# alvin-zyl/LDDL

Measured on AMD Instinct MI355X. Metric: WordPiece tokens/sec (node) BERT seq128/512 at 1-8 GPUs; % HBM roofline, higher is better.
Workload: dtype u8

## Files before the change

lddl_amd/csrc/capi.hip:

```cpp
#include "capi_ctx.h"

static thread_local char g_err[1024];

int set_err(int code, const char* fmt, ...) {
  va_list ap;
  va_start(ap, fmt);
  vsnprintf(g_err, sizeof g_err, fmt, ap);
  va_end(ap);
  return code;
}

extern "C" const char* lddl_last_error(void) { return g_err; }

static void free_ctx(lddl_ctx* c) {
  if (!c) return;
  (void)hipFree(c->d_tdbg);
  (void)hipFree(c->d_pdbg);
  (void)hipFree(c->d_top);
  (void)hipFree(c->d_pages);
  (void)hipFree(c->d_bmp);
  (void)hipFree(c->d_xmap);
  (void)hipFree(c->d_multi);
  (void)hipFree(c->d_slots);
  (void)hipFree(c->d_bloom);
// ... 149 lines not shown
}

extern "C" int lddl_tokenize_stats(lddl_ctx* c, double* out, int n) {
  if (!c || !out || n < 6) return set_err(LDDL_EINVAL, "need out[6]");
  if (!c->timing || !c->tm) return set_err(LDDL_EINVAL, "timing is off (lddl_set_timing)");
  HIP_TRY(hipSetDevice(c->device));
  for (int k = 0; k < 3; ++k) {
    double ms = 0.0;
    for (int i = 0; i < c->tm->n[k]; ++i) {
      HIP_TRY(hipEventSynchronize(c->tm->ev[k][1][i]));
      float f = 0.0f;
      HIP_TRY(hipEventElapsedTime(&f, c->tm->ev[k][0][i], c->tm->ev[k][1][i]));
      ms += f;
    }
    out[k] = ms;
  }
  unsigned long long nrec = 0;
  HIP_TRY(hipMemcpy(&nrec, c->d_nrec, 8, hipMemcpyDeviceToHost));
  out[3] = (double)nrec;
  out[4] = (double)c->tm->n[0];
  uint32_t nfb = 0;
  HIP_TRY(hipMemcpy(&nfb, c->d_counter + 8, 4, hipMemcpyDeviceToHost));
  out[5] = (double)nfb;
  return 0;
}
```

lddl_amd/csrc/capi_ctx.h:

```cpp
#pragma once
#include <hip/hip_runtime.h>

#include <stdarg.h>
#include <stdint.h>
#include <stdio.h>
#include <stdlib.h>
#include <string.h>

#include <algorithm>
#include <new>
#include <string>
#include <vector>

#include "../../include/lddl_amd.h"
#include "collate.h"
#include "common.h"
#include "pack.h"
#include "render.h"
#include "tok_tables.h"
#include "tokenize.h"

using namespace lddl;

__attribute__((visibility("hidden"))) int set_err(int code, const char* fmt, ...);
// ... 45 lines not shown

enum CtxWs {
  CW_BIN_HIST,
  CW_BIN_BASE,
  CW_BIN_BSUM,
  CW_BIN_ERR,
  CW_NPY_ERR,
  CW_TILE_SENT,
  CW_FB_LIST,
  CW_FB_COUNT,
  CW_ENT,
  CW_SHARED_ROWS,
  CW_SHARED_BSUM,
  CW_SHARED_META,
  CW_COLLATE_ERR,
  CW_SENT_SPEC,
  CW_PCS,
  CW_SNSLOT,
  CW_CNT8,
  CW_SCAN_BSUM,
  CW_PCH,
  CW_CHUNK_PART,
  CW_PART_PB,
  CW_COUNT
};

enum HostWord {
  HW_NPAIRS,
  HW_BART_LO = HW_NPAIRS,
  HW_NTOK,
  HW_BART_HI = HW_NTOK,
  HW_PACK_ERR,
  HW_BART_NSENT = HW_PACK_ERR,
  HW_NMASK,
  HW_MARENA_USED,
  HW_NDENSE,
  HW_CU_TOTAL = HW_NDENSE,
  HW_MAX_LEN,
  HW_RENDER_BYTES = HW_MAX_LEN,
  HW_ERR,
  HW_COUNT
};
static_assert(HW_MAX_LEN == HW_CU_TOTAL + 1, "lddl_collate_rows_cu_seqlens reads total and max_len with one copy");
static_assert(HW_PACK_ERR == HW_NTOK + 1 && HW_NMASK == HW_NTOK + 2, "lddl_rows_from_strings_len reads its three totals with one copy");

struct lddl_pack {
  int device = 0;
  WsBuf ws[PW_COUNT];
  PackParams pp{};
  int64_t last_npairs = -1, last_ntok = -1, last_nmask = -1, last_ndense = 0;
  int pack_codebert = 0;
  uint64_t mlm_cap = 0;
  uint16_t* last_tokens = nullptr;
// ... 18 lines not shown
  uint8_t* d_pool = nullptr;
  uint32_t* d_voff = nullptr;
  uint8_t* d_rpool = nullptr;
  uint32_t* d_rinfo = nullptr;
  uint32_t maxb[2] = {0, 0};
  uint4* d_vt = nullptr;
  uint32_t vt_mask = 0;
  uint32_t* d_vbloom = nullptr;
  bool scan_ok = false;
  bool timing = false;
  SplitTiming* tm = nullptr;
  unsigned long long* d_nrec = nullptr;
  const void* spec_ids = nullptr;
  const void* spec_ntok = nullptr;
  const void* spec_soff = nullptr;
  int64_t spec_nsent = -1;
  bool spec_flags = false;
  WsBuf ws[CW_COUNT];
  int64_t* h_tot = nullptr;
  lddl_pack own;
  uint64_t mlm_cap0 = 0;
  int tok_grid = 0;
  int tok_algo = 5;
  uint8_t* d_ovf = nullptr;
  uint32_t* d_counter = nullptr;
  uint64_t* d_tdbg = nullptr;
  uint64_t* d_pdbg = nullptr;
  int64_t pdbg_cap = 0;
  uint2* d_ctab = nullptr;
  uint32_t ctab_mask = 0;
};

template <class T>
static int ws_get(WsBuf* ws, int slot, size_t n, T** out) {
  auto& b = ws[slot];
  const size_t bytes = (n ? n : 1) * sizeof(T);
  if (b.cap < bytes) {
    (void)hipFree(b.p);
    b.p = nullptr;
    b.cap = 0;
    HIP_TRY(hipMalloc(&b.p, bytes));
    b.cap = bytes;
  }
  *out = (T*)b.p;
  return 0;
}
// ... 29 lines not shown
```

lddl_amd/csrc/capi_tokenize.hip:

```cpp
#include "capi_ctx.h"

static int tok_debug_report(const TokParams& P, int64_t nt, hipStream_t st) {
  uint64_t h[24];
  HIP_TRY(hipMemcpyAsync(h, P.dbg, sizeof h, hipMemcpyDeviceToHost, st));
  HIP_TRY(hipStreamSynchronize(st));
  const char* nm[12] = {"loop", "setup", "classify", "except", "units", "urec", "prep", "probe", "records",
                        "tile_end", "entries", "tiles"};
  fprintf(stderr, "[lddl tok5 dbg] ntiles=%lld", (long long)nt);
  for (int k = 0; k < 12; ++k) fprintf(stderr, " %s=%llu", nm[k], (unsigned long long)h[k]);
  const char* wn[6] = {"wp_A", "wp_B", "wp_C", "wp_D", "wp_steps", "wp_lane_steps"};
  for (int k = 0; k < 6; ++k) fprintf(stderr, " %s=%llu", wn[k], (unsigned long long)h[12 + k]);
  fprintf(stderr, " prep_decode=%llu prep_dirty=%llu x_list=%llu x_load=%llu x_apply=%llu", (unsigned long long)h[18],
          (unsigned long long)h[19], (unsigned long long)h[20], (unsigned long long)h[21], (unsigned long long)h[22]);
  fprintf(stderr, "\n");
  return 0;
}

extern "C" int lddl_tokenize(lddl_ctx* c, const uint8_t* d_bytes, int64_t nbytes, const int64_t* d_sent_off,
                             int64_t n_sent, int32_t max_tok, uint16_t* d_out_ids, int64_t out_cap,
                             int32_t* d_out_ntok, int64_t* d_out_tok_off, void* stream) {
  if (!c) return set_err(LDDL_EINVAL, "null ctx");
  if (n_sent < 0 || max_tok < 1 || max_tok > 65534 || nbytes < 0 || out_cap < 0)
    return set_err(LDDL_EINVAL, "n_sent %lld nbytes %lld max_tok %d out_cap %lld", (long long)n_sent,
                   (long long)nbytes, max_tok, (long long)out_cap);
// ... 34 lines not shown
  P.bloom = c->d_bloom;
  P.pool = c->d_pool;
  P.voff = c->d_voff;
  P.maxb[0] = c->maxb[0];
  P.maxb[1] = c->maxb[1];
  for (int k = 0; k < 5; ++k) P.special[k] = c->special[k];
  P.unk = c->special[1];
  P.vt = c->d_vt;
  P.vt_mask = c->vt_mask;
  P.vbloom = c->d_vbloom;
  P.ovf = c->d_ovf;
  P.work_counter = c->d_counter;
  HIP_TRY(hipMemsetAsync(c->d_counter, 0, 64, st));
  const char* dbgenv = getenv("LDDL_TOK_DEBUG");

  if (dbgenv && dbgenv[0] == '1') {
    if (!c->d_tdbg) HIP_TRY(hipMalloc((void**)&c->d_tdbg, 32 * 8));
    HIP_TRY(hipMemsetAsync(c->d_tdbg, 0, 32 * 8, st));
    P.dbg = c->d_tdbg;
  }
  const int64_t nt = tile_count(nbytes);
  const char* eseg = getenv("LDDL_SPLIT_SEG");
  const char* ech = getenv("LDDL_SPLIT_CHUNKS");
  const int64_t seg_max = c->tok_algo == 0 ? nt : eseg && atoll(eseg) > 0 ? atoll(eseg) : SPLIT_SEG_TILES;
  const int64_t seg = nt < seg_max ? nt : seg_max;
  const bool split = c->tok_algo == 5;
  int64_t n_chunks = !split ? 1 : split_seg_slots(seg, c->n_cu) / SPLIT_CHUNK;
  if (ech && atoll(ech) > 0 && split) n_chunks = atoll(ech);
  const int64_t slots = n_chunks * SPLIT_CHUNK;
  int64_t* tile_sent;
  SplitParams S{};
  int rc;
  const int64_t fb_cap = fb_list_cap(seg, n_sent);
  if ((rc = ws_get(c, CW_TILE_SENT, nt + 1, &tile_sent)) || (rc = ws_get(c, CW_FB_LIST, (size_t)(2 * fb_cap), &S.fb_list)) ||
      (rc = ws_get(c, CW_FB_COUNT, 16, &S.fb_count)) ||
      (rc = ws_get(c, CW_ENT, (size_t)seg * 1024 + (size_t)max_tok + 4096, &S.ent)) ||
      (rc = ws_get(c, CW_SHARED_BSUM, (size_t)n_chunks + 16, &S.chunk_fill)) ||
      (rc = ws_get(c, CW_SCAN_BSUM, (size_t)scan_blocks(n_sent) + 1, &S.scan_bsum)))
    return rc;
  if ((rc = ws_get(c, CW_SHARED_ROWS, (size_t)slots * 4, &S.rec)) || (rc = ws_get(c, CW_PCS, (size_t)slots * 4, &S.pcs)) ||
      (rc = ws_get(c, CW_PCH, (size_t)slots, &S.pch)) || (rc = ws_get(c, CW_SHARED_META, n_sent, &S.smeta)) ||
      (rc = ws_get(c, CW_SNSLOT, n_sent, &S.snslot)) || (rc = ws_get(c, CW_CNT8, (size_t)slots, &S.cnt8)))
    return rc;
  if (!S.pch || !S.smeta || !S.snslot || !S.cnt8 || !S.rec || !S.pcs)
    return set_err(LDDL_EINVAL, "tokenize: finish scratch not allocated");
  S.chunk_ctr = S.chunk_fill + n_chunks;
  S.n_chunks = (uint32_t)n_chunks;
  S.seg_tiles = seg;
  S.fb_cap = fb_cap;
  S.seg_sent_cap = n_sent;
  S.n_fallback = c->d_counter + 8;
  if (c->timing) {
    S.n_rec = c->d_nrec;
    HIP_TRY(hipMemsetAsync(c->d_nrec, 0, 8, st));
  }
  if (c->tok_algo == 0) {
    HIP_TRY(launch_tokenize_serial_dense(P, nbytes, tile_sent, S, c->n_cu, c->tok_grid, st));
  } else {
    HIP_TRY(launch_tokenize_split(P, nbytes, tile_sent, S, c->n_cu, c->tok_grid, st,
                                  c->timing ? c->tm : nullptr));
  }
  if (P.dbg) return tok_debug_report(P, nt, st);
  return 0;
}
```

lddl_amd/csrc/tokenize.h:

```cpp
#pragma once
#include <hip/hip_runtime.h>
#include <stdint.h>

namespace lddl {

constexpr int WB_OVF = 384;
constexpr int TOK_WAVES = 4;
constexpr int BLOOM_WORDS = 8192;

struct TokParams {
  const uint8_t* bytes;
  const int64_t* sent_off;
  int64_t n_sent;
  int32_t max_tok;
  uint16_t* out_ids;
  int32_t* out_ntok;
  int64_t* out_tok_off;
  int64_t out_cap;
  uint8_t* sent_spec;
  const uint16_t* top;
  const uint32_t* pages;
  const uint4* multi;
  const uint32_t* bmp;
  const uint32_t* xmap;
// ... 5 lines not shown
  uint32_t maxb[2];
  uint32_t special[5];
  uint32_t unk;
  const uint4* vt;
  uint32_t vt_mask;
  const uint32_t* vbloom;
  uint8_t* ovf;
  uint32_t* work_counter;
  uint64_t* dbg;
};

int64_t tile_count(int64_t nbytes);
hipError_t launch_tile_bounds(const int64_t* sent_off, int64_t n_sent, int64_t n_tiles, int64_t* tile_sent,
                              hipStream_t s, int64_t seg = 0, int sup = 1);
hipError_t launch_tokenize_fallback(const TokParams& P, const int64_t* fb_list, const int32_t* fb_count,
                                    int64_t fb_cap, int grid, hipStream_t s);
const void* tokenize_fallback_kernel_ptr();
hipError_t launch_list_all_tiles(int64_t n_tiles, const int64_t* tile_sent, int64_t* fb_list, int32_t* fb_count,
                                 int64_t fb_cap, hipStream_t s);
inline int64_t fb_list_cap(int64_t seg_tiles, int64_t n_sent) {
  return 2 * seg_tiles + 64 + (n_sent + 30) / 31;
}

constexpr int64_t SPLIT_SEG_TILES = int64_t(1) << 23;
constexpr uint32_t SPLIT_CHUNK = 1024;
constexpr uint32_t SPLIT_EDEF = 0xF000u;
constexpr uint16_t SPLIT_NENT_FB = 0xFFFFu;
constexpr uint16_t SPLIT_EHOLE = 0xFFFFu;

struct SplitParams {
  int64_t seg_tiles;
  int64_t t0, t1;
  const int64_t* tile_sent;
  uint16_t* ent;
  uint4* rec;
  uint4* pcs;
  uint4* pch;
  uint32_t* chunk_fill;
  uint32_t* chunk_ctr;
  uint32_t n_chunks;
  uint2* smeta;
  uint16_t* snslot;
  uint8_t* cnt8;
  int64_t* scan_bsum;
  int64_t seg_sent_cap;
  int64_t* fb_list;
  int32_t* fb_count;
  int64_t fb_cap;
  uint32_t* n_fallback;
  unsigned long long* n_rec;
};
struct SplitTiming {
  hipEvent_t ev[3][2][64];
  int n[3];
};
hipError_t launch_tokenize_split(const TokParams& P, int64_t nbytes, int64_t* tile_sent, SplitParams S, int n_cu,
                                 int fb_grid, hipStream_t s, SplitTiming* tm = nullptr);
hipError_t launch_tokenize_serial_dense(const TokParams& P, int64_t nbytes, int64_t* tile_sent, SplitParams S,
                                        int n_cu, int fb_grid, hipStream_t s);
int64_t split_seg_slots(int64_t seg_tiles, int n_cu);

}
```

lddl_amd/csrc/tokenize_split.hip:

```cpp
#include <string.h>

#include "common.h"
#include "tokenize.h"
#include "wave.h"
#include "tokenize_serial.h"
#include "pack.h"


namespace lddl {
namespace tok5 {

constexpr int CAP = 2048;
constexpr int DCAP = 256;
constexpr int SCAN_OCC = 5;
#ifndef LDDL_SCAN_SUPER
#define LDDL_SCAN_SUPER 16
#endif
constexpr int SUPER = LDDL_SCAN_SUPER;
#ifndef LDDL_SCAN_FK
#define LDDL_SCAN_FK 2
#endif
constexpr int FK = LDDL_SCAN_FK;
#ifndef LDDL_SCAN_FKEY
#define LDDL_SCAN_FKEY 16
// ... 253 lines not shown
        else if (cls == CLS_SPACE) c |= C_S;
        else if (cls == CLS_ISOLATE) c |= C_I;
        else c |= C_W;
        if (kind == KIND_MAP && cls == CLS_OTHER) c |= C_UP;
        if (b == '[') c |= C_X;
      } else {
        c = b >= 0xC0 ? (C_X | C_CS) : 0u;
      }
      word |= c << (8 * k);
    }
    ctab32[threadIdx.x] = word;
  }
  __syncthreads();
  const uint8_t* ctab = reinterpret_cast<const uint8_t*>(ctab32);
  const int lane = threadIdx.x & 63;
  const int wv = __builtin_amdgcn_readfirstlane(threadIdx.x >> 6);
  Lds& L = Ls[wv];
  const int64_t base = P.sent_off[0];
  const int64_t ebase = S.t0 << 10;
  const int64_t nwaves = (int64_t)gridDim.x * WAVES;
  const int max_tok = P.max_tok;
  uint32_t cur = 0, cend = 0, cbase = 0, tbase = 0, tsl = 0;
  int chunk = -1;
  int64_t n_sa = 0, n_sb = 0, n_A = 0, n_B = 0;
  int nst = 0;
  bool dma_pending = false;
  const int64_t ng = (S.t1 - S.t0 + SUPER - 1) / SUPER;
  auto dma4 = [&](const void* g, uint32_t* l) { lds_dma4(g, l); };
  auto drain = [&]() { asm volatile("s_waitcnt vmcnt(0)" ::: "memory"); };
  auto st_bounds = [&](int64_t g) {
    if (g < ng && lane < 4) {
      const int64_t t = min(S.t1, S.t0 + (g + (lane >> 1)) * SUPER);
      dma4(reinterpret_cast<const uint32_t*>(S.tile_sent + t) + (lane & 1), L.pb);
    }
  };
  uint32_t* const sctr = S.chunk_ctr + 2;
  uint32_t gq = 0;
  auto claim = [&]() {
    if (lane == 0) gq = atomicAdd(sctr, 1u);
  };
  {
    const int64_t g = (int64_t)blockIdx.x * WAVES + wv;
    int64_t cs = 0, ce = 0, gn = ng;
    if (g < ng) {
      cs = uni64(S.tile_sent[S.t0 + g * SUPER]);
      ce = uni64(S.tile_sent[min(S.t1, S.t0 + (g + 1) * SUPER)]);
// ... 579 lines not shown
          if (len > 0 && len <= 24) key = load_key(L.nb, src, len);
          if (len > 0) {
            const uint32_t b0 = key.d0 & 0xFFu;
            if (!dirty && len <= 24 && b0 >= BS && b0 < BS + 5) {
              id = (uint16_t)P.special[b0 - BS];
            } else if (len > 100 && count_chars(L.nb, src, len) > 100) {
              id = (uint16_t)P.unk;
            } else {
              id = U_DEFER;
              w = 1;
              lovf |= len > KEYMAX;
            }
          }
          STAMP(6);
          if (w != 0 && !miss && len <= 24 && len <= mb0) {
            const uint32_t hk = key_hash(key, len, 0u), want = ((uint32_t)len << 16) | 0x80000000u;
            const uint4* bk = P.vt + 4 * (hk & vmask);
            const uint4 fa = bk[0], fb = bk[1];
            if (slot_eq(fa, fb, key, want)) {
              id = (uint16_t)(fb.z & 0xFFFFu);
              w = 0;
            }
          }
          if (__any(lovf)) {
            ovf = true;
            break;
          }
          STAMP(7);
          const uint32_t nsl = (valid && id == U_DEFER) ? (len <= KEY1 ? 1u : 2u) : 0u;
          const uint64_t N1 = __ballot(nsl != 0), N2 = __ballot(nsl == 2);
          const uint32_t need = (uint32_t)(__popcll(N1) + __popcll(N2));
          if (need > 0 && cur + need > cend) {
            if (tsl + need > SPLIT_CHUNK) {
              ovf = true;
              break;
            }
            if (chunk >= 0 && lane == 0) S.chunk_fill[chunk] = tbase - cbase;
            int c = 0;
            if (lane == 0) c = (int)atomicAdd(S.chunk_ctr, 1u);
            c = __builtin_amdgcn_readfirstlane(c);
            if ((uint32_t)c >= S.n_chunks) {
              chunk = -1;
              cur = cend = cbase = tbase = 0;
              ovf = true;
              break;
            }
            chunk = c;
            cbase = (uint32_t)c * SPLIT_CHUNK;
            cend = cbase + SPLIT_CHUNK;
            if (tsl) {
              asm volatile("s_waitcnt vmcnt(0)" ::: "memory");
              for (int k = 0; k < 4; ++k)
                for (uint32_t i = lane; i < tsl; i += 64) *recq(S, k, cbase + i) = *recq(S, k, tbase + i);
              for (uint32_t i = lane; i < tsl; i += 64) S.cnt8[cbase + i] = 0;
            }
            tbase = cbase;
            cur = cbase + tsl;
          }
          STAMP(10);
          const uint32_t o = tsl + (uint32_t)(lane_rank(N1) + lane_rank(N2));
          if (valid) {
            S.ent[ent0 + (int)L.ebs[sj] + rb + u] =
                (uint16_t)(id == U_EMPTY ? SPLIT_EHOLE : id != U_DEFER ? id : (SPLIT_EDEF | o));
            if (id == U_EMPTY || id == U_DEFER) atomicAdd(&L.sacc[sj], nsl | 0x10000u);
            else if (id == P.special[2] || id == P.special[3]) atomicOr(&L.sspec[sj >> 5], 1u << (sj & 31));
          }
          if (nsl) {
            const uint32_t slot = tbase + o;
            uint32_t kd[6] = {key.d0, key.d1, key.d2, key.d3, key.d4, key.d5};
            const int a = src >> 2;
            const uint32_t sh = (uint32_t)(src & 3);
            if (len > 24) {
              uint32_t xx[7];
#pragma unroll
              for (int i = 0; i < 7; ++i) xx[i] = L.nb[a + i];
#pragma unroll
              for (int i = 0; i < 6; ++i) kd[i] = __builtin_amdgcn_alignbyte(xx[i + 1], xx[i], sh);
            }
            *recq(S, 0, slot) = make_uint4((uint32_t)len | (nsl << 8) | 0x80000000u, 0u, kd[0], kd[1]);
            *recq(S, 1, slot) = make_uint4(kd[2], kd[3], kd[4], kd[5]);
            if (len > 24) {
              uint32_t xx[9];
#pragma unroll
              for (int i = 0; i < 9; ++i) xx[i] = L.nb[a + 6 + i];
              uint32_t kq[8];
#pragma unroll
              for (int i = 0; i < 8; ++i) kq[i] = keep_bytes(__builtin_amdgcn_alignbyte(xx[i + 1], xx[i], sh), len - 24 - 4 * i);
              *recq(S, 2, slot) = make_uint4(kq[0], kq[1], kq[2], kq[3]);
              *recq(S, 3, slot) = make_uint4(kq[4], kq[5], kq[6], kq[7]);
            }
            if (nsl == 2) {
              *recq(S, 0, slot + 1) = make_uint4(0, 0, 0, 0);
              S.cnt8[slot + 1] = 0;
            }
          }
          tsl += need;
          cur += need;
          wsync();
          STAMP(8);
        }
      }
      if (ovf) break;
    }
    if (ovf) {
      fallback();
      return;
    }
    {
      const uint32_t acc = lane < ns ? L.sacc[lane] : 0u;
      const uint32_t nsl = acc & 0xFFFFu;
      const uint32_t sq0 = wave_incl_add(nsl) - nsl;
      if (lane < ns) {
// ... 98 lines not shown
    const uint32_t h = l >= 12 ? H3 : vmix(vmix(vmix(VSEED, vmask_rem(c0, l)), vmask_rem(c1, l - 4)), vmask_rem(c2, l - 8));
    return vfinal(h, (uint32_t)l, cont);
  };
  auto bkey_len = [&](int l) {
    const int lc = min(l, 24), q = lc >> 2, rr = lc & 3;
    return vbkey(selH(q), rr ? selD(q) & ((1u << (8 * rr)) - 1u) : 0u, (uint32_t)l, cont);
  };
  auto bloom_ok = [&](uint32_t h) {
    const uint32_t bb = vbloom_bits(h);
    return (bloom[vbloom_word(h)] & bb) == bb;
  };
  auto shrink = [&]() {
    --e;
    if (!(asc && e - s < 24))
      while (e > s && (kbyte(e) & 0xC0u) == 0x80u) --e;
  };
  auto start_piece = [&](int maxb) {
    bslot = -1;
    load_cand();
    e = min(we, s + maxb);
    if (e < we && !(asc && e - s < 24))
      while (e > s && (kbyte(e) & 0xC0u) == 0x80u) --e;
  };
  uint4* const outs = S.pcs;
  auto rec16 = [&]() { return reinterpret_cast<uint16_t*>(outs + (size_t)r * 4); };
  uint32_t pw01 = 0, pw23 = 0;
  auto put_piece = [&](int k, uint32_t id) {
    if (k < 4) {
      const uint32_t sh = 16u * (uint32_t)(k & 1);
      const uint32_t keep = ~(0xFFFFu << sh), val = id << sh;
      if (k < 2) pw01 = (pw01 & keep) | val;
      else pw23 = (pw23 & keep) | val;
    } else {
      rec16()[piece_at(k)] = (uint16_t)id;
    }
  };
  auto finish = [&]() {
    S.pch[r] = make_uint4((uint32_t)np, pw01, pw23, 0u);
    S.cnt8[r] = (uint8_t)np;
    r = -1;
  };
  uint64_t wacc[6] = {0, 0, 0, 0, 0, 0}, wprev = 0;
  const bool wdbg = P.dbg != nullptr;
#define WP_STAMP(k)                                                              \
  if (wdbg) {                                                                    \
    uint64_t t_;                                                                 \
    asm volatile("s_memtime %0\n\ts_waitcnt lgkmcnt(0)" : "=s"(t_)::"memory"); \
    wacc[k] += t_ - wprev;                                                       \
    wprev = t_;                                                                  \
  }
  if (wdbg) asm volatile("s_memtime %0\n\ts_waitcnt lgkmcnt(0)" : "=s"(wprev)::"memory");
  for (;;) {
    bool fail = false;
    uint4 a0 = make_uint4(0, 0, 0, 0), a1 = a0, b0 = a0, b1 = a0;
    if (r >= 0) {
      if (bslot < 0) {
        int len = e - s;
        bool found = false;
        uint32_t hcur = 0;
        if (len <= 24) {
          int fl = 0;
// ... 79 lines not shown
        };
        const uint32_t m0c = msk(0, c0), m1c = msk(1, c1), m2c = msk(2, c2), m3c = msk(3, c3), m4c = msk(4, c4),
                       m5c = msk(5, c5);
        const uint32_t want = ((uint32_t)len << 16) | (cont << 24) | 0x80000000u;
        bool m0 = (((a1.z & 0xFFFF0000u) ^ want) | (a0.x ^ m0c) | (a0.y ^ m1c) | (a0.z ^ m2c) | (a0.w ^ m3c) |
                   (a1.x ^ m4c) | (a1.y ^ m5c)) == 0u;
        bool m1 = (((b1.z & 0xFFFF0000u) ^ want) | (b0.x ^ m0c) | (b0.y ^ m1c) | (b0.z ^ m2c) | (b0.w ^ m3c) |
                   (b1.x ^ m4c) | (b1.y ^ m5c)) == 0u;
        if (len > 24) {
          if (m0)
            for (int k = 24; k < len; ++k) m0 = m0 && kbyte(s + k) == P.pool[a1.w + k];
          if (m1)
            for (int k = 24; k < len; ++k) m1 = m1 && kbyte(s + k) == P.pool[b1.w + k];
        }
        if (m0 || m1) {
          put_piece(np, (m0 ? a1.z : b1.z) & 0xFFFFu);
          ++np;
          s = e;
          if (s >= we) {
            finish();
          } else {
            cont = 1;
            start_piece(mb1);
          }
        } else if (!(a1.z & 0x80000000u) || !(b1.z & 0x80000000u)) {
          bslot = -1;
          shrink();
        } else {
          bslot = (int)(((uint32_t)bslot + 1u) & vmask);
        }
      }
    }
    WP_STAMP(2)
    if (pr >= 0) {
      if (q0.x == 0u) {
        pr = -1;
      } else if ((q0.x & 0xFFu) > 24u && !qlong) {
        q2 = *recq(S, 2, (uint32_t)pr);
        q3 = *recq(S, 3, (uint32_t)pr);
        qlong = true;
      } else if (r < 0) {
        const int len = (int)(q0.x & 0xFFu);
        kb[0] = q0.z; kb[64] = q0.w;
        kb[128] = q1.x; kb[192] = q1.y; kb[256] = q1.z; kb[320] = q1.w;
        kb[384] = q2.x; kb[448] = q2.y; kb[512] = q2.z; kb[576] = q2.w;
        kb[640] = q3.x; kb[704] = q3.y; kb[768] = q3.z; kb[832] = q3.w;
        kb[896] = 0u;
        kb[960] = 0u;
        r = pr;
        pr = -1;
        ++nrec;
        s = 0;
        we = len;
        np = 0;
        cont = 0;
        start_piece(mb0);
      }
    }
    WP_STAMP(3)
    if (wdbg) {
      wacc[4] += 1;
      wacc[5] += __popcll(__ballot(r >= 0));
// ... 42 lines not shown
struct ExpSent {
  int64_t eb;
  int64_t dst;
  uint32_t qb;
  uint32_t lim;
  uint32_t e0;
  uint32_t pad;
};
struct ExpLds {
  ExpSent sn[64];
  uint32_t hf[64];
};

template <bool ALL_DIRECT>
__global__ __launch_bounds__(256) void expand_kernel(TokParams P, SplitParams S) {
  __shared__ ExpLds X[4];
  const int lane = threadIdx.x & 63;
  const int wv = __builtin_amdgcn_readfirstlane(threadIdx.x >> 6);
  ExpLds& E = X[wv];
  const int64_t sA = uni64(S.tile_sent[S.t0]), sB = uni64(S.tile_sent[S.t1]);
  const int64_t base = P.sent_off[0], ebase = S.t0 << 10;
  const int64_t nwaves = (int64_t)gridDim.x * 4;
  typedef uint32_t u32x3 __attribute__((ext_vector_type(3)));
  const uint4* const pcs = S.pcs;
  const uint4* const pch = S.pch;
  uint32_t tag = 0;
  E.hf[lane] = 0u;
  for (int64_t g0 = sA + ((int64_t)blockIdx.x * 4 + wv) * 64; g0 < sB; g0 += nwaves * 64) {
    const int64_t s = g0 + lane;
    uint32_t ne = 0;
    int64_t eoff = 0, d = 0;
    uint32_t qb = 0, lim = 0;
    if (s < sB) {
      const uint2 m = S.smeta[s];
      const int32_t nt = P.out_ntok[s];
      ne = m.x & 0xFFFFu;
      if (ne == SPLIT_NENT_FB) ne = (uint32_t)nt;
      d = P.out_tok_off[s];
      eoff = P.sent_off[s] - base - ebase;
      qb = (m.x & 0xFFFFu) == SPLIT_NENT_FB ? 0u : m.y;
      lim = (uint32_t)max((int64_t)0, min((int64_t)nt, P.out_cap - d));
    }
    const uint32_t x = wave_incl_add(ne);
    const uint32_t e0 = x - ne;
    const uint32_t T = lane_get(x, 63);
    ExpSent es;
    es.eb = eoff - (int64_t)e0;
// ... 33 lines not shown
          const uint32_t g = st + (uint32_t)lane;
          xj[k] = min(owner(st), 63u);
          xin[k] = g < T;
          const ExpSent sj = E.sn[xj[k]];
          xv[k] = S.ent[xin[k] ? sj.eb + g : 0];
        }
      }
      u32x3 xr[EXP_K];
#pragma unroll
      for (int k = 0; k < EXP_K; ++k) {
        const bool r = !ALL_DIRECT && xin[k] && xv[k] >= SPLIT_EDEF && xv[k] != SPLIT_EHOLE;
        xr[k] = u32x3{0u, 0u, 0u};
        if (st0 + 64 * k < T)
          xr[k] = *reinterpret_cast<const u32x3*>(pch + (r ? (size_t)(E.sn[xj[k]].qb + (xv[k] & 0xFFFu)) : 0));
      }
#pragma unroll
      for (int k = 0; k < EXP_K; ++k) {
        const uint32_t st = st0 + 64 * k;
        if (st >= T) break;
        const uint32_t cj = xj[k], cv = xin[k] ? xv[k] : 0u;
        const bool cin = xin[k], rec = !ALL_DIRECT && cin && cv >= SPLIT_EDEF && cv != SPLIT_EHOLE;
        const u32x3 rq = rec ? xr[k] : u32x3{cin && (ALL_DIRECT || cv != SPLIT_EHOLE) ? 1u : 0u, 0u, 0u};
        const ExpSent sj = E.sn[cj];
        const size_t ri = (size_t)(sj.qb + (cv & 0xFFFu)) * 4;
        const uint32_t cnt = rq.x;
        const uint32_t xex = wave_incl_add(cnt) - cnt;
        const int hl = (int)(sj.e0 - st);
        const uint32_t hb = (uint32_t)__shfl((int)xex, hl & 63);
        const uint32_t p = xex - (hl >= 0 ? hb : 0u - carry);
        const int room = (int)sj.lim - (int)p;
        const uint32_t nw = room > 0 ? min(cnt, (uint32_t)room) : 0u;
        if (nw) {
          uint16_t* o = P.out_ids + sj.dst + p;
          o[0] = (uint16_t)(ALL_DIRECT || cv < SPLIT_EDEF ? cv : rq.y & 0xFFFFu);
          if (nw > 1) o[1] = (uint16_t)(rq.y >> 16);
          if (nw > 2) o[2] = (uint16_t)(rq.z & 0xFFFFu);
          if (nw > 3) o[3] = (uint16_t)(rq.z >> 16);
          if (nw > 4) {
            const uint16_t* pc = reinterpret_cast<const uint16_t*>(pcs + ri);
            for (uint32_t q = 4; q < nw; ++q) o[q] = pc[piece_at((int)q)];
          }
        }
        const uint32_t ll = min(T, st + 64) - 1 - st;
        carry = lane_get(p + cnt, (int)ll);
      }
    }
    wsync();
  }
}

template <int WAVES, bool DBG, int OCC>
static hipError_t launch_scan(const TokParams& P, const SplitParams& S, int n_cu, hipStream_t s) {
  static int per_cu = 0;
  if (per_cu == 0 &&
      (hipOccupancyMaxActiveBlocksPerMultiprocessor(&per_cu, scan_kernel<WAVES, DBG, OCC>, 64 * WAVES, 0) !=
           hipSuccess ||
       per_cu < 1))
    per_cu = 1;
  int64_t grid = (int64_t)n_cu * per_cu;
  const int64_t ng = (S.t1 - S.t0 + SUPER - 1) / SUPER;
  const int64_t need = (ng + WAVES - 1) / WAVES;
  if (grid > need) grid = need;
  if (grid < 1) grid = 1;
  hipLaunchKernelGGL((scan_kernel<WAVES, DBG, OCC>), dim3((unsigned)grid), dim3(64 * WAVES), 0, s, P, S);
  return hipGetLastError();
}

template <int WAVES>
static hipError_t launch_wp(const TokParams& P, const SplitParams& S, int n_cu, hipStream_t s) {
  static int per_cu = 0;
  if (per_cu == 0 &&
      (hipOccupancyMaxActiveBlocksPerMultiprocessor(&per_cu, wp_kernel<WAVES>, 64 * WAVES, 0) != hipSuccess ||
       per_cu < 1))
    per_cu = 1;
  const int64_t grid = (int64_t)n_cu * per_cu;
  hipLaunchKernelGGL(wp_kernel<WAVES>, dim3((unsigned)grid), dim3(64 * WAVES), 0, s, P, S);
  return hipGetLastError();
}

}

constexpr int SCAN_WAVES = 4, WP_WAVES = 12;
hipError_t finish_segment(TokParams P, const SplitParams& S, int n_cu, int fb_grid, hipStream_t s, bool all_direct = false);

int64_t split_seg_slots(int64_t seg_tiles, int n_cu) {
  int per_cu = 0;
  if (hipOccupancyMaxActiveBlocksPerMultiprocessor(&per_cu, tok5::scan_kernel<SCAN_WAVES, false, tok5::SCAN_OCC>, 64 * SCAN_WAVES,
                                                   0) != hipSuccess || per_cu < 1)
    per_cu = 8;
  const int64_t waves = (int64_t)n_cu * per_cu * SCAN_WAVES;
  const int64_t chunks = (seg_tiles * 1024 / 14 + SPLIT_CHUNK - 1) / SPLIT_CHUNK + std::min(waves, seg_tiles) + 16;
  return chunks * SPLIT_CHUNK;
}

__global__ void smeta_fallback_kernel(uint2* smeta, int64_t n_sent) {
  for (int64_t s = (int64_t)blockIdx.x * blockDim.x + threadIdx.x; s < n_sent; s += (int64_t)gridDim.x * blockDim.x)
    smeta[s] = make_uint2(SPLIT_NENT_FB, 0xFFFFFFFFu);
}

hipError_t launch_tokenize_serial_dense(const TokParams& P, int64_t nbytes, int64_t* tile_sent, SplitParams S,
                                        int n_cu, int fb_grid, hipStream_t s) {
  const int64_t n_tiles = tile_count(nbytes);
  hipError_t e = launch_tile_bounds(P.sent_off, P.n_sent, n_tiles, tile_sent, s);
  if (e != hipSuccess || (e = hipMemsetAsync(P.out_tok_off, 0, sizeof(int64_t), s)) != hipSuccess) return e;
  S.tile_sent = tile_sent;
  S.t0 = 0;
  S.t1 = n_tiles;
  if ((e = launch_list_all_tiles(n_tiles, tile_sent, S.fb_list, S.fb_count, S.fb_cap, s)) != hipSuccess) return e;
  hipLaunchKernelGGL(smeta_fallback_kernel, dim3(1024), dim3(256), 0, s, S.smeta, P.n_sent);
  if ((e = hipGetLastError()) != hipSuccess) return e;
  return finish_segment(P, S, n_cu, fb_grid, s, true);
}

hipError_t launch_tokenize_split(const TokParams& P, int64_t nbytes, int64_t* tile_sent, SplitParams S, int n_cu,
                                 int fb_grid, hipStream_t s, SplitTiming* tm) {
  if (tm) tm->n[0] = tm->n[1] = tm->n[2] = 0;
  auto mark = [&](int k, int side) -> hipError_t {
    if (!tm || tm->n[k] >= 64) return hipSuccess;
    const hipError_t e = hipEventRecord(tm->ev[k][side][tm->n[k]], s);
    if (side == 1) ++tm->n[k];
    return e;
  };
  const int64_t n_tiles = tile_count(nbytes);
  const int64_t seg = S.seg_tiles > 0 ? S.seg_tiles : SPLIT_SEG_TILES;
  hipError_t e = launch_tile_bounds(P.sent_off, P.n_sent, n_tiles, tile_sent, s, seg, tok5::SUPER);
  if (e != hipSuccess) return e;
  if ((e = hipMemsetAsync(P.out_tok_off, 0, sizeof(int64_t), s)) != hipSuccess) return e;
  S.tile_sent = tile_sent;
  for (int64_t t0 = 0; t0 < n_tiles; t0 += seg) {
    S.t0 = t0;
    S.t1 = std::min(n_tiles, t0 + seg);
    if ((e = hipMemsetAsync(S.chunk_ctr, 0, 12, s)) != hipSuccess) return e;
    if ((e = hipMemsetAsync(S.fb_count, 0, 4, s)) != hipSuccess) return e;
    if ((e = mark(0, 0)) != hipSuccess) return e;
    if (P.dbg) e = tok5::launch_scan<SCAN_WAVES, true, tok5::SCAN_OCC>(P, S, n_cu, s);
    else e = tok5::launch_scan<SCAN_WAVES, false, tok5::SCAN_OCC>(P, S, n_cu, s);
    if (e != hipSuccess || (e = mark(0, 1)) != hipSuccess || (e = mark(1, 0)) != hipSuccess) return e;
    if ((e = tok5::launch_wp<WP_WAVES>(P, S, n_cu, s)) != hipSuccess) return e;
    if ((e = mark(1, 1)) != hipSuccess || (e = mark(2, 0)) != hipSuccess) return e;
    if ((e = finish_segment(P, S, n_cu, fb_grid, s)) != hipSuccess || (e = mark(2, 1)) != hipSuccess) return e;
  }
  return hipSuccess;
}

hipError_t finish_segment(TokParams P, const SplitParams& S, int n_cu, int fb_grid, hipStream_t s, bool all_direct) {
  TokParams F = P;
  F.out_ids = S.ent - (S.t0 << 10);
  hipError_t e = launch_tokenize_fallback(F, S.fb_list, S.fb_count, S.fb_cap, fb_grid, s);
  if (e != hipSuccess) return e;
#ifndef LDDL_CNT_BLOCKS
#define LDDL_CNT_BLOCKS 256
#endif
  const int64_t cnt_grid = std::max<int64_t>(
      1, std::min<int64_t>((int64_t)n_cu * LDDL_CNT_BLOCKS, (S.seg_sent_cap + 256 * tok5::CNT_U - 1) / (256 * tok5::CNT_U)));
  hipLaunchKernelGGL(tok5::count_kernel, dim3((unsigned)cnt_grid), dim3(256), 0, s, P, S);
// ... 17 lines not shown
```

lddl_amd/tokenizer.py:

```python
import ctypes

import numpy as np
import torch

from . import _lib

_WHITE_SPACE = ''.join(map(chr, list(range(0x09, 0x0E)) + [0x20, 0x85, 0xA0, 0x1680] + list(range(0x2000, 0x200B)) +
                           [0x2028, 0x2029, 0x202F, 0x205F, 0x3000]))
TOKENS_MAX = 65534


def _ptr(t):
  return ctypes.c_void_p(t.data_ptr()) if t is not None else ctypes.c_void_p(0)


def _stream(stream=None):
  s = stream if stream is not None else torch.cuda.current_stream()
  return ctypes.c_void_p(s.cuda_stream)


class CapacityError(RuntimeError):

  def __init__(self, total, cap):
    super().__init__('lddl_amd: %d token ids do not fit the %d-entry ids buffer' % (total, cap))
# ... 60 lines not shown
    if cap < nbytes:
      total = self.total_tokens(out_tok_off, n_sent, stream)
      if total > cap:
        raise CapacityError(total, cap)
    return out_ids, out_ntok, out_tok_off

  @staticmethod
  def total_tokens(tok_off, n_sent, stream=None):
    (stream if stream is not None else torch.cuda.current_stream()).synchronize()
    return int(tok_off[n_sent].item())

  def set_special_flags(self, on=True):
    _lib.check(_lib.lib().lddl_set_special_flags(self.handle, 1 if on else 0))

  def set_algo(self, algo):
    out = ctypes.c_int(-1)
    _lib.check(_lib.lib().lddl_set_tokenize_algo(self.handle, int(algo), ctypes.byref(out)))
    return out.value

  def set_timing(self, on=True):
    _lib.check(_lib.lib().lddl_set_timing(self.handle, 1 if on else 0))

  def stats(self):
    out = (ctypes.c_double * 6)()
    _lib.check(_lib.lib().lddl_tokenize_stats(self.handle, out, 6))
    return {'scan_ms': out[0], 'wordpiece_ms': out[1], 'expand_ms': out[2], 'records': int(out[3]),
            'launches': int(out[4]), 'fallback_tiles': int(out[5])}

  def encode_batch(self, sentences, max_tok=512):
    enc = [s.encode('utf-8') for s in sentences]
    off = np.zeros(len(enc) + 1, dtype=np.int64)
    np.cumsum([len(b) for b in enc], out=off[1:])
    raw = np.frombuffer(b''.join(enc) + b'\0' * 16, dtype=np.uint8)
    d = torch.from_numpy(raw.copy()).to(self.device)
    o = torch.from_numpy(off).to(self.device)
    ids, ntok, toff = self.tokenize_device(d, o, max_tok)
    ids = ids.cpu().numpy().view(np.uint16)
    toff = toff.cpu().numpy()
    return [ids[toff[i]:toff[i + 1]].astype(np.int64).tolist() for i in range(len(enc))]

  def tokenize(self, text, max_length=512, truncation=True, **kwargs):
    cap = max_length if truncation else TOKENS_MAX
    ids = self.encode_batch([text], cap)[0]
    if not truncation and len(ids) >= TOKENS_MAX:
      raise ValueError('lddl_amd: text reaches %d tokens; truncation=False cannot return it whole' % TOKENS_MAX)
    return [self.ids_to_tokens[i] for i in ids]

  def convert_tokens_to_ids(self, tokens):
    return [self.vocab.get(t, self.unk_id) for t in tokens]
```

Measured before the change: 46.32 billion.

## Compact split-tokenizer records with pooled long-key and piece storage and budgeted segments

Shrinks per-slot record storage from four to two uint4 rows. Long-key tails and pieces beyond four now go into separately sized pools, handed out in blocks by atomic wave-level claims, with a serial rerun if the pieces pool overflows. Segment size is now picked by binary search against a share of free device memory, up to a larger maximum, instead of a fixed constant. The aim is less scratch memory traffic and fewer segments per call. In exchange it adds atomics, two extra host word fetches and an error read per call, and a costly fallback path on pool overflow.

```diff
diff --git a/lddl_amd/csrc/capi.hip b/lddl_amd/csrc/capi.hip
--- a/lddl_amd/csrc/capi.hip
+++ b/lddl_amd/csrc/capi.hip
@@ -195,5 +195,10 @@
   uint32_t nfb = 0;
   HIP_TRY(hipMemcpy(&nfb, c->d_counter + 8, 4, hipMemcpyDeviceToHost));
   out[5] = (double)nfb;
-  return 0;
-}
+  if (n >= 9) {
+    out[6] = (double)c->tok_serial_reruns;
+    out[7] = (double)c->tok_pool_used[0];
+    out[8] = (double)c->tok_pool_used[1];
+  }
+  return 0;
+}
diff --git a/lddl_amd/csrc/capi_ctx.h b/lddl_amd/csrc/capi_ctx.h
--- a/lddl_amd/csrc/capi_ctx.h
+++ b/lddl_amd/csrc/capi_ctx.h
@@ -91,13 +91,16 @@
   CW_PCH,
   CW_CHUNK_PART,
   CW_PART_PB,
+  CW_LONGKEY,
   CW_COUNT
 };
 
 enum HostWord {
   HW_NPAIRS,
+  HW_TOK_LONGKEYS = HW_NPAIRS,
   HW_BART_LO = HW_NPAIRS,
   HW_NTOK,
+  HW_TOK_PIECES = HW_NTOK,
   HW_BART_HI = HW_NTOK,
   HW_PACK_ERR,
   HW_BART_NSENT = HW_PACK_ERR,
@@ -162,6 +165,9 @@
   uint64_t mlm_cap0 = 0;
   int tok_grid = 0;
   int tok_algo = 5;
+  int64_t tok_budget = -1;
+  uint32_t tok_pool_used[2] = {0, 0};
+  int64_t tok_serial_reruns = 0;
   uint8_t* d_ovf = nullptr;
   uint32_t* d_counter = nullptr;
   uint64_t* d_tdbg = nullptr;
diff --git a/lddl_amd/csrc/capi_tokenize.hip b/lddl_amd/csrc/capi_tokenize.hip
--- a/lddl_amd/csrc/capi_tokenize.hip
+++ b/lddl_amd/csrc/capi_tokenize.hip
@@ -80,30 +80,53 @@
   const int64_t nt = tile_count(nbytes);
   const char* eseg = getenv("LDDL_SPLIT_SEG");
   const char* ech = getenv("LDDL_SPLIT_CHUNKS");
-  const int64_t seg_max = c->tok_algo == 0 ? nt : eseg && atoll(eseg) > 0 ? atoll(eseg) : SPLIT_SEG_TILES;
-  const int64_t seg = nt < seg_max ? nt : seg_max;
+  const char* elk = getenv("LDDL_SPLIT_LONGKEYS");
+  const char* epp = getenv("LDDL_SPLIT_PIECES");
   const bool split = c->tok_algo == 5;
+  if (split && c->tok_budget < 0) {
+    size_t free_b = 0, total_b = 0;
+    HIP_TRY(hipMemGetInfo(&free_b, &total_b));
+    c->tok_budget = (int64_t)(free_b / 100) * SPLIT_MEM_SHARE_PCT;
+  }
+  const int64_t seg_max = !split ? nt
+                          : eseg && atoll(eseg) > 0 ? atoll(eseg)
+                                                     : split_choose_seg(nt, split_scan_waves(c->n_cu), c->tok_budget);
+  const int64_t seg = std::max<int64_t>(1, nt < seg_max ? nt : seg_max);
   int64_t n_chunks = !split ? 1 : split_seg_slots(seg, c->n_cu) / SPLIT_CHUNK;
   if (ech && atoll(ech) > 0 && split) n_chunks = atoll(ech);
   const int64_t slots = n_chunks * SPLIT_CHUNK;
+  int64_t n_lk = split_pool_cap(slots, 0), n_pp = split_pool_cap(slots, 1);
+  if (elk && elk[0] && atoll(elk) >= 0) n_lk = atoll(elk);
+  if (epp && epp[0] && atoll(epp) >= 0) n_pp = atoll(epp);
   int64_t* tile_sent;
   SplitParams S{};
   int rc;
   const int64_t fb_cap = fb_list_cap(seg, n_sent);
+  if (slots >= (int64_t(1) << 31) || fb_cap >= (int64_t(1) << 31) || n_lk >= (int64_t(1) << 31) ||
+      n_pp >= (int64_t(1) << 31) - 2)
+    return set_err(LDDL_EINVAL,
+                   "tokenize: a segment of %lld tiles needs %lld record slots, %lld ranges, %lld long-key and %lld pieces "
+                   "pool entries: one of them passes 2^31 (LDDL_SPLIT_SEG / _CHUNKS / _LONGKEYS / _PIECES)",
+                   (long long)seg, (long long)slots, (long long)fb_cap, (long long)n_lk, (long long)n_pp);
   if ((rc = ws_get(c, CW_TILE_SENT, nt + 1, &tile_sent)) || (rc = ws_get(c, CW_FB_LIST, (size_t)(2 * fb_cap), &S.fb_list)) ||
       (rc = ws_get(c, CW_FB_COUNT, 16, &S.fb_count)) ||
       (rc = ws_get(c, CW_ENT, (size_t)seg * 1024 + (size_t)max_tok + 4096, &S.ent)) ||
       (rc = ws_get(c, CW_SHARED_BSUM, (size_t)n_chunks + 16, &S.chunk_fill)) ||
       (rc = ws_get(c, CW_SCAN_BSUM, (size_t)scan_blocks(n_sent) + 1, &S.scan_bsum)))
     return rc;
-  if ((rc = ws_get(c, CW_SHARED_ROWS, (size_t)slots * 4, &S.rec)) || (rc = ws_get(c, CW_PCS, (size_t)slots * 4, &S.pcs)) ||
+  if ((rc = ws_get(c, CW_SHARED_ROWS, (size_t)slots * 2, &S.rec)) ||
+      (rc = ws_get(c, CW_PCS, ((size_t)n_pp + 2) * 4, &S.ppool)) ||
+      (rc = ws_get(c, CW_LONGKEY, (size_t)std::max<int64_t>(n_lk, 1) * 2, &S.lkp)) ||
       (rc = ws_get(c, CW_PCH, (size_t)slots, &S.pch)) || (rc = ws_get(c, CW_SHARED_META, n_sent, &S.smeta)) ||
       (rc = ws_get(c, CW_SNSLOT, n_sent, &S.snslot)) || (rc = ws_get(c, CW_CNT8, (size_t)slots, &S.cnt8)))
     return rc;
-  if (!S.pch || !S.smeta || !S.snslot || !S.cnt8 || !S.rec || !S.pcs)
+  if (!S.pch || !S.smeta || !S.snslot || !S.cnt8 || !S.rec || !S.ppool || !S.lkp)
     return set_err(LDDL_EINVAL, "tokenize: finish scratch not allocated");
   S.chunk_ctr = S.chunk_fill + n_chunks;
   S.n_chunks = (uint32_t)n_chunks;
+  S.n_lk = (uint32_t)n_lk;
+  S.n_pp = (uint32_t)n_pp;
+  S.pp_ovf = c->d_counter + 9;
   S.seg_tiles = seg;
   S.fb_cap = fb_cap;
   S.seg_sent_cap = n_sent;
@@ -117,6 +140,21 @@
   } else {
     HIP_TRY(launch_tokenize_split(P, nbytes, tile_sent, S, c->n_cu, c->tok_grid, st,
                                   c->timing ? c->tm : nullptr));
+    HIP_TRY(fetch_word(c, HW_TOK_LONGKEYS, S.chunk_ctr + 3, 4, st));
+    HIP_TRY(fetch_word(c, HW_TOK_PIECES, S.chunk_ctr + 4, 4, st));
+    uint32_t ovf = 0;
+    if ((rc = read_err(c, S.pp_ovf, st, &ovf))) return rc;
+    c->tok_pool_used[0] = (uint32_t)(c->h_tot[HW_TOK_LONGKEYS] & 0xFFFFFFFF);
+    c->tok_pool_used[1] = (uint32_t)(c->h_tot[HW_TOK_PIECES] & 0xFFFFFFFF);
+    const char* epl = getenv("LDDL_SPLIT_POOLS");
+    if (epl && epl[0] == '1')
+      fprintf(stderr, "[lddl split pools] bytes=%lld seg_tiles=%lld slots=%lld longkeys=%u/%lld pieces=%u/%lld overflow=%u\n",
+              (long long)nbytes, (long long)seg, (long long)slots, c->tok_pool_used[0], (long long)n_lk,
+              c->tok_pool_used[1], (long long)n_pp, ovf);
+    if (ovf) {
+      ++c->tok_serial_reruns;
+      HIP_TRY(launch_tokenize_serial_dense(P, nbytes, tile_sent, S, c->n_cu, c->tok_grid, st));
+    }
   }
   if (P.dbg) return tok_debug_report(P, nt, st);
   return 0;
diff --git a/lddl_amd/csrc/tokenize.h b/lddl_amd/csrc/tokenize.h
--- a/lddl_amd/csrc/tokenize.h
+++ b/lddl_amd/csrc/tokenize.h
@@ -51,7 +51,12 @@
   return 2 * seg_tiles + 64 + (n_sent + 30) / 31;
 }
 
-constexpr int64_t SPLIT_SEG_TILES = int64_t(1) << 23;
+constexpr int64_t SPLIT_SEG_TILES_MAX = int64_t(24) << 20;
+constexpr int64_t SPLIT_SEG_TILES_MIN = int64_t(1) << 20;
+constexpr int64_t SPLIT_SLOT_BYTES = 14;
+constexpr int64_t SPLIT_LK_DIV = 32;
+constexpr int64_t SPLIT_PP_DIV = 32;
+constexpr int SPLIT_MEM_SHARE_PCT = 65;
 constexpr uint32_t SPLIT_CHUNK = 1024;
 constexpr uint32_t SPLIT_EDEF = 0xF000u;
 constexpr uint16_t SPLIT_NENT_FB = 0xFFFFu;
@@ -63,8 +68,11 @@
   const int64_t* tile_sent;
   uint16_t* ent;
   uint4* rec;
-  uint4* pcs;
+  uint4* lkp;
+  uint4* ppool;
   uint4* pch;
+  uint32_t n_lk, n_pp;
+  uint32_t* pp_ovf;
   uint32_t* chunk_fill;
   uint32_t* chunk_ctr;
   uint32_t n_chunks;
@@ -88,5 +96,39 @@
 hipError_t launch_tokenize_serial_dense(const TokParams& P, int64_t nbytes, int64_t* tile_sent, SplitParams S,
                                         int n_cu, int fb_grid, hipStream_t s);
 int64_t split_seg_slots(int64_t seg_tiles, int n_cu);
+int64_t split_scan_waves(int n_cu);
+
+constexpr int64_t SPLIT_CHUNK_I = 1024;
+inline int64_t split_slots_for(int64_t seg_tiles, int64_t scan_waves) {
+  const int64_t chunks = (seg_tiles * 1024 / SPLIT_SLOT_BYTES + SPLIT_CHUNK_I - 1) / SPLIT_CHUNK_I +
+                         (scan_waves < seg_tiles ? scan_waves : seg_tiles) + 16;
+  return chunks * SPLIT_CHUNK_I;
+}
+constexpr int64_t SPLIT_LK_BLOCK = 64, SPLIT_PP_BLOCK = 128;
+constexpr int64_t SPLIT_POOL_WAVES = int64_t(1) << 20;
+inline int64_t split_pool_cap(int64_t slots, int which) {
+  const int64_t div = which == 0 ? SPLIT_LK_DIV : SPLIT_PP_DIV;
+  return (slots + div - 1) / div + SPLIT_POOL_WAVES;
+}
+inline int64_t split_seg_scratch_bytes(int64_t seg_tiles, int64_t scan_waves) {
+  const int64_t slots = split_slots_for(seg_tiles, scan_waves);
+  return seg_tiles * 2048 + slots * 49 + slots / SPLIT_CHUNK_I * 4 + split_pool_cap(slots, 0) * 32 +
+         (split_pool_cap(slots, 1) + 2) * 64 + 16 * (2 * seg_tiles + 64);
+}
+inline int64_t split_choose_seg(int64_t n_tiles, int64_t scan_waves, int64_t budget) {
+  if (n_tiles <= 1) return 1;
+  const int64_t hi0 = n_tiles < SPLIT_SEG_TILES_MAX ? n_tiles : SPLIT_SEG_TILES_MAX;
+  int64_t lo = hi0 < SPLIT_SEG_TILES_MIN ? hi0 : SPLIT_SEG_TILES_MIN, hi = hi0;
+  while (lo < hi) {
+    const int64_t mid = lo + (hi - lo + 1) / 2;
+    if (split_seg_scratch_bytes(mid, scan_waves) <= budget) lo = mid;
+    else hi = mid - 1;
+  }
+  const int64_t n_seg = (n_tiles + lo - 1) / lo;
+  return (n_tiles + n_seg - 1) / n_seg;
+}
+static_assert(SPLIT_SEG_TILES_MAX * 1024 / SPLIT_SLOT_BYTES + (int64_t(1) << 26) < (int64_t(1) << 31),
+              "record slots of the largest segment (+ 64 Ki partly used chunks) must stay below 2^31");
+static_assert(SPLIT_SEG_TILES_MAX / 16 < (int64_t(1) << 21), "super-tiles of a segment: the scan's u32 claim counter");
 
 }
diff --git a/lddl_amd/csrc/tokenize_split.hip b/lddl_amd/csrc/tokenize_split.hip
--- a/lddl_amd/csrc/tokenize_split.hip
+++ b/lddl_amd/csrc/tokenize_split.hip
@@ -299,6 +299,9 @@
   const int max_tok = P.max_tok;
   uint32_t cur = 0, cend = 0, cbase = 0, tbase = 0, tsl = 0;
   int chunk = -1;
+  constexpr uint32_t LK_BLOCK = (uint32_t)SPLIT_LK_BLOCK;
+  uint32_t lkcur = 0, lkend = 0;
+  bool lkdry = false;
   int64_t n_sa = 0, n_sb = 0, n_A = 0, n_B = 0;
   int nst = 0;
   bool dma_pending = false;
@@ -924,6 +927,26 @@
               w = 0;
             }
           }
+          uint32_t lki = 0;
+          const bool lkw = w != 0 && len > 24 && len <= KEYMAX;
+          const uint64_t LK = __ballot(lkw);
+          if (LK != 0) {
+            const uint32_t nlk = (uint32_t)__popcll(LK);
+            if (lkcur + nlk > lkend && !lkdry) {
+              uint32_t b = 0;
+              if (lane == 0) b = atomicAdd(S.chunk_ctr + 3, LK_BLOCK);
+              b = (uint32_t)__builtin_amdgcn_readfirstlane((int)b);
+              lkcur = min(b, S.n_lk);
+              lkend = lkcur + min(S.n_lk - lkcur, LK_BLOCK);
+              lkdry = lkend - lkcur < LK_BLOCK;
+            }
+            if (lkcur + nlk > lkend) {
+              lovf = true;
+            } else {
+              lki = lkw ? lkcur + (uint32_t)lane_rank(LK) : 0u;
+              lkcur += nlk;
+            }
+          }
           if (__any(lovf)) {
             ovf = true;
             break;
@@ -952,7 +975,7 @@
             cend = cbase + SPLIT_CHUNK;
             if (tsl) {
               asm volatile("s_waitcnt vmcnt(0)" ::: "memory");
-              for (int k = 0; k < 4; ++k)
+              for (int k = 0; k < 2; ++k)
                 for (uint32_t i = lane; i < tsl; i += 64) *recq(S, k, cbase + i) = *recq(S, k, tbase + i);
               for (uint32_t i = lane; i < tsl; i += 64) S.cnt8[cbase + i] = 0;
             }
@@ -979,7 +1002,7 @@
 #pragma unroll
               for (int i = 0; i < 6; ++i) kd[i] = __builtin_amdgcn_alignbyte(xx[i + 1], xx[i], sh);
             }
-            *recq(S, 0, slot) = make_uint4((uint32_t)len | (nsl << 8) | 0x80000000u, 0u, kd[0], kd[1]);
+            *recq(S, 0, slot) = make_uint4((uint32_t)len | (nsl << 8) | 0x80000000u, lki, kd[0], kd[1]);
             *recq(S, 1, slot) = make_uint4(kd[2], kd[3], kd[4], kd[5]);
             if (len > 24) {
               uint32_t xx[9];
@@ -988,8 +1011,8 @@
               uint32_t kq[8];
 #pragma unroll
               for (int i = 0; i < 8; ++i) kq[i] = keep_bytes(__builtin_amdgcn_alignbyte(xx[i + 1], xx[i], sh), len - 24 - 4 * i);
-              *recq(S, 2, slot) = make_uint4(kq[0], kq[1], kq[2], kq[3]);
-              *recq(S, 3, slot) = make_uint4(kq[4], kq[5], kq[6], kq[7]);
+              S.lkp[2 * (size_t)lki] = make_uint4(kq[0], kq[1], kq[2], kq[3]);
+              S.lkp[2 * (size_t)lki + 1] = make_uint4(kq[4], kq[5], kq[6], kq[7]);
             }
             if (nsl == 2) {
               *recq(S, 0, slot + 1) = make_uint4(0, 0, 0, 0);
@@ -1134,8 +1157,11 @@
     if (e < we && !(asc && e - s < 24))
       while (e > s && (kbyte(e) & 0xC0u) == 0x80u) --e;
   };
-  uint4* const outs = S.pcs;
-  auto rec16 = [&]() { return reinterpret_cast<uint16_t*>(outs + (size_t)r * 4); };
+  constexpr uint32_t PP_DRY = 0xFFFFFFFFu, PP_BLOCK = (uint32_t)SPLIT_PP_BLOCK;
+  uint32_t ppi = 0;
+  uint32_t ppcur = 0, ppend = 0;
+  bool ppdry = false, wantc = false;
+  auto rec16 = [&]() { return reinterpret_cast<uint16_t*>(S.ppool + (size_t)ppi * 4); };
   uint32_t pw01 = 0, pw23 = 0;
   auto put_piece = [&](int k, uint32_t id) {
     if (k < 4) {
@@ -1144,11 +1170,11 @@
       if (k < 2) pw01 = (pw01 & keep) | val;
       else pw23 = (pw23 & keep) | val;
     } else {
-      rec16()[piece_at(k)] = (uint16_t)id;
+      if (ppi != PP_DRY) rec16()[piece_at(k)] = (uint16_t)id;
     }
   };
   auto finish = [&]() {
-    S.pch[r] = make_uint4((uint32_t)np, pw01, pw23, 0u);
+    S.pch[r] = make_uint4((uint32_t)np, pw01, pw23, np > 4 && ppi != PP_DRY ? ppi : 0u);
     S.cnt8[r] = (uint8_t)np;
     r = -1;
   };
@@ -1274,6 +1300,7 @@
           } else {
             cont = 1;
             start_piece(mb1);
+            wantc = np == 4;
           }
         } else if (!(a1.z & 0x80000000u) || !(b1.z & 0x80000000u)) {
           bslot = -1;
@@ -1283,13 +1310,36 @@
         }
       }
     }
+    {
+      const uint64_t CM = __ballot(wantc);
+      if (CM != 0) {
+        const uint64_t C2 = __ballot(wantc && we > KEY1);
+        const uint32_t need = (uint32_t)(__popcll(CM) + __popcll(C2));
+        if (ppcur + need > ppend && !ppdry) {
+          uint32_t b = 0;
+          if (lane == 0) b = atomicAdd(S.chunk_ctr + 4, PP_BLOCK);
+          b = (uint32_t)__builtin_amdgcn_readfirstlane((int)b);
+          ppcur = min(b, S.n_pp);
+          ppend = ppcur + min(S.n_pp - ppcur, PP_BLOCK);
+          ppdry = ppend - ppcur < PP_BLOCK;
+        }
+        const bool got = ppcur + need <= ppend;
+        if (wantc) {
+          ppi = got ? ppcur + (uint32_t)(lane_rank(CM) + lane_rank(C2)) : PP_DRY;
+          if (!got && lane_rank(CM) == 0) atomicOr(S.pp_ovf, 1u);
+          wantc = false;
+        }
+        if (got) ppcur += need;
+      }
+    }
     WP_STAMP(2)
     if (pr >= 0) {
       if (q0.x == 0u) {
         pr = -1;
       } else if ((q0.x & 0xFFu) > 24u && !qlong) {
-        q2 = *recq(S, 2, (uint32_t)pr);
-        q3 = *recq(S, 3, (uint32_t)pr);
+        const size_t lk = 2 * (size_t)min(q0.y, max(S.n_lk, 1u) - 1u);
+        q2 = S.lkp[lk];
+        q3 = S.lkp[lk + 1];
         qlong = true;
       } else if (r < 0) {
         const int len = (int)(q0.x & 0xFFu);
@@ -1378,7 +1428,6 @@
   const int64_t base = P.sent_off[0], ebase = S.t0 << 10;
   const int64_t nwaves = (int64_t)gridDim.x * 4;
   typedef uint32_t u32x3 __attribute__((ext_vector_type(3)));
-  const uint4* const pcs = S.pcs;
   const uint4* const pch = S.pch;
   uint32_t tag = 0;
   E.hf[lane] = 0u;
@@ -1458,7 +1507,7 @@
         const bool cin = xin[k], rec = !ALL_DIRECT && cin && cv >= SPLIT_EDEF && cv != SPLIT_EHOLE;
         const u32x3 rq = rec ? xr[k] : u32x3{cin && (ALL_DIRECT || cv != SPLIT_EHOLE) ? 1u : 0u, 0u, 0u};
         const ExpSent sj = E.sn[cj];
-        const size_t ri = (size_t)(sj.qb + (cv & 0xFFFu)) * 4;
+        const size_t ri = (size_t)(sj.qb + (cv & 0xFFFu));
         const uint32_t cnt = rq.x;
         const uint32_t xex = wave_incl_add(cnt) - cnt;
         const int hl = (int)(sj.e0 - st);
@@ -1473,7 +1522,8 @@
           if (nw > 2) o[2] = (uint16_t)(rq.z & 0xFFFFu);
           if (nw > 3) o[3] = (uint16_t)(rq.z >> 16);
           if (nw > 4) {
-            const uint16_t* pc = reinterpret_cast<const uint16_t*>(pcs + ri);
+            const uint32_t pe = min(pch[ri].w, S.n_pp);
+            const uint16_t* pc = reinterpret_cast<const uint16_t*>(S.ppool + (size_t)pe * 4);
             for (uint32_t q = 4; q < nw; ++q) o[q] = pc[piece_at((int)q)];
           }
         }
@@ -1520,14 +1570,18 @@
 hipError_t finish_segment(TokParams P, const SplitParams& S, int n_cu, int fb_grid, hipStream_t s, bool all_direct = false);
 
 int64_t split_seg_slots(int64_t seg_tiles, int n_cu) {
-  int per_cu = 0;
-  if (hipOccupancyMaxActiveBlocksPerMultiprocessor(&per_cu, tok5::scan_kernel<SCAN_WAVES, false, tok5::SCAN_OCC>, 64 * SCAN_WAVES,
-                                                   0) != hipSuccess || per_cu < 1)
+  return split_slots_for(seg_tiles, split_scan_waves(n_cu));
+}
+
+int64_t split_scan_waves(int n_cu) {
+  static int per_cu = 0;
+  if (per_cu == 0 &&
+      (hipOccupancyMaxActiveBlocksPerMultiprocessor(&per_cu, tok5::scan_kernel<SCAN_WAVES, false, tok5::SCAN_OCC>,
+                                                    64 * SCAN_WAVES, 0) != hipSuccess || per_cu < 1))
     per_cu = 8;
-  const int64_t waves = (int64_t)n_cu * per_cu * SCAN_WAVES;
-  const int64_t chunks = (seg_tiles * 1024 / 14 + SPLIT_CHUNK - 1) / SPLIT_CHUNK + std::min(waves, seg_tiles) + 16;
-  return chunks * SPLIT_CHUNK;
-}
+  return (int64_t)n_cu * per_cu * SCAN_WAVES;
+}
+static_assert(SPLIT_CHUNK == SPLIT_CHUNK_I, "the host sizing functions' chunk");
 
 __global__ void smeta_fallback_kernel(uint2* smeta, int64_t n_sent) {
   for (int64_t s = (int64_t)blockIdx.x * blockDim.x + threadIdx.x; s < n_sent; s += (int64_t)gridDim.x * blockDim.x)
@@ -1537,15 +1591,19 @@
 hipError_t launch_tokenize_serial_dense(const TokParams& P, int64_t nbytes, int64_t* tile_sent, SplitParams S,
                                         int n_cu, int fb_grid, hipStream_t s) {
   const int64_t n_tiles = tile_count(nbytes);
+  const int64_t seg = S.seg_tiles > 0 ? S.seg_tiles : n_tiles;
   hipError_t e = launch_tile_bounds(P.sent_off, P.n_sent, n_tiles, tile_sent, s);
   if (e != hipSuccess || (e = hipMemsetAsync(P.out_tok_off, 0, sizeof(int64_t), s)) != hipSuccess) return e;
   S.tile_sent = tile_sent;
-  S.t0 = 0;
-  S.t1 = n_tiles;
-  if ((e = launch_list_all_tiles(n_tiles, tile_sent, S.fb_list, S.fb_count, S.fb_cap, s)) != hipSuccess) return e;
   hipLaunchKernelGGL(smeta_fallback_kernel, dim3(1024), dim3(256), 0, s, S.smeta, P.n_sent);
   if ((e = hipGetLastError()) != hipSuccess) return e;
-  return finish_segment(P, S, n_cu, fb_grid, s, true);
+  for (int64_t t0 = 0; t0 < n_tiles; t0 += seg) {
+    S.t0 = t0;
+    S.t1 = std::min(n_tiles, t0 + seg);
+    if ((e = launch_list_all_tiles(S.t1 - S.t0, tile_sent + t0, S.fb_list, S.fb_count, S.fb_cap, s)) != hipSuccess) return e;
+    if ((e = finish_segment(P, S, n_cu, fb_grid, s, true)) != hipSuccess) return e;
+  }
+  return hipSuccess;
 }
 
 hipError_t launch_tokenize_split(const TokParams& P, int64_t nbytes, int64_t* tile_sent, SplitParams S, int n_cu,
@@ -1558,7 +1616,7 @@
     return e;
   };
   const int64_t n_tiles = tile_count(nbytes);
-  const int64_t seg = S.seg_tiles > 0 ? S.seg_tiles : SPLIT_SEG_TILES;
+  const int64_t seg = S.seg_tiles > 0 ? S.seg_tiles : n_tiles;
   hipError_t e = launch_tile_bounds(P.sent_off, P.n_sent, n_tiles, tile_sent, s, seg, tok5::SUPER);
   if (e != hipSuccess) return e;
   if ((e = hipMemsetAsync(P.out_tok_off, 0, sizeof(int64_t), s)) != hipSuccess) return e;
@@ -1566,7 +1624,7 @@
   for (int64_t t0 = 0; t0 < n_tiles; t0 += seg) {
     S.t0 = t0;
     S.t1 = std::min(n_tiles, t0 + seg);
-    if ((e = hipMemsetAsync(S.chunk_ctr, 0, 12, s)) != hipSuccess) return e;
+    if ((e = hipMemsetAsync(S.chunk_ctr, 0, 20, s)) != hipSuccess) return e;
     if ((e = hipMemsetAsync(S.fb_count, 0, 4, s)) != hipSuccess) return e;
     if ((e = mark(0, 0)) != hipSuccess) return e;
     if (P.dbg) e = tok5::launch_scan<SCAN_WAVES, true, tok5::SCAN_OCC>(P, S, n_cu, s);
diff --git a/lddl_amd/tokenizer.py b/lddl_amd/tokenizer.py
--- a/lddl_amd/tokenizer.py
+++ b/lddl_amd/tokenizer.py
@@ -106,10 +106,11 @@
     _lib.check(_lib.lib().lddl_set_timing(self.handle, 1 if on else 0))
 
   def stats(self):
-    out = (ctypes.c_double * 6)()
-    _lib.check(_lib.lib().lddl_tokenize_stats(self.handle, out, 6))
+    out = (ctypes.c_double * 9)()
+    _lib.check(_lib.lib().lddl_tokenize_stats(self.handle, out, 9))
     return {'scan_ms': out[0], 'wordpiece_ms': out[1], 'expand_ms': out[2], 'records': int(out[3]),
-            'launches': int(out[4]), 'fallback_tiles': int(out[5])}
+            'launches': int(out[4]), 'fallback_tiles': int(out[5]), 'serial_reruns': int(out[6]),
+            'longkey_used': int(out[7]), 'pieces_used': int(out[8])}
 
   def encode_batch(self, sentences, max_tok=512):
     enc = [s.encode('utf-8') for s in sentences]
```

New measurement: 46.66 billion, median of 6. No clear change (+0.7%).
